# Guillaume-Helbecque/GPU-accelerated-tree-search-Chapel

Hardware: NVIDIA H100
Metric: Mnodes/s (higher is better)
Workload: dtype u8

## Files before the change

### gpu-accelerated-tree-search-chapel_b200/csrc/nq_rounds_ll.cuh

```cuda
#pragma once
#include "ll_tiers.h"
#include "nq_kernel.cuh"

namespace tsb {

constexpr int LL_T = 256;
__host__ __device__ constexpr int ll_slice(int ppt) { return LL_T * ppt; }
static_assert(ll_slice(2) == LL_SLICE2 && ll_slice(3) == LL_SLICE3, "ll_tiers.h");

enum { RND_EXIT_DONE = 0, RND_EXIT_PAUSE = 1, RND_EXIT_SPACE = 2, RND_EXIT_ABORT = 3, RND_EXIT_RELAUNCH = 4 };
struct RoundsState {
  long long size;
  unsigned epoch;
  int exit_code;
  unsigned long long rounds, parents, children, solutions;
  long long prof[12];
  long long size_hi;
  unsigned long long t_start, t_exit;
  unsigned cta_sm[LL_MAX_SMS], cta_t0[LL_MAX_SMS];
  unsigned cta_fertile[LL_MAX_SMS], cta_wide[LL_MAX_SMS];
};
__device__ __forceinline__ unsigned long long ll_globaltimer() {
  unsigned long long t;
  asm volatile("mov.u64 %0, %%globaltimer;" : "=l"(t));
  return t;
}
__device__ __forceinline__ unsigned ll_smid() {
  unsigned s;
  asm volatile("mov.u32 %0, %%smid;" : "=r"(s));
  return s;
}

__device__ __forceinline__ void st_relaxed_u64(unsigned long long* p, unsigned long long v) {
  asm volatile("st.relaxed.gpu.global.u64 [%0], %1;" ::"l"(p), "l"(v) : "memory");
}
struct SpinGuard {
  unsigned spins = 0;
  long long t0 = 0;
  __device__ __forceinline__ bool expired(unsigned* abort_flag) {
    if ((++spins & 0xFFu) != 0) return false;
    if (*reinterpret_cast<volatile unsigned*>(abort_flag)) return true;
    const long long now = clock64();
    if (t0 == 0) t0 = now;
    if (now - t0 > 4000000000LL) {
      *reinterpret_cast<volatile unsigned*>(abort_flag) = 1u;
      return true;
    }
    return false;
  }
};
constexpr int LL_CAP = 2048;
constexpr int LL_WORDS = 4;
constexpr int LL_LAYERS = 1024;
constexpr unsigned LL_TRUSTED = 0u;
__device__ __forceinline__ unsigned ll_tag(unsigned e) { return e % LL_TAG_SPAN + 1u; }

struct alignas(32) FatNode {
  unsigned long long w[LL_WORDS];
};
__device__ __forceinline__ void ll_piece(uint32_t d0, uint32_t d1, uint32_t mask, uint32_t tag, unsigned long long& a,
                                         unsigned long long& b) {
  a = static_cast<unsigned long long>(__byte_perm(mask, tag, 0x5410)) << 32 | d0;
  b = static_cast<unsigned long long>(__byte_perm(mask, tag, 0x5432)) << 32 | d1;
}
constexpr int LL_CM_SHIFT = 10;
constexpr uint32_t LL_LEAF = 1u << 30;
__host__ __device__ constexpr int ll_fw(int i) { return i / 6; }
__host__ __device__ constexpr int ll_fs(int i) { return 5 * (i % 6); }
__device__ __forceinline__ uint32_t ll_depth(uint32_t d0, uint32_t d1, uint32_t d2) {
  return d0 >> 30 | (d1 >> 30) << 2 | (d2 >> 30) << 4;
}
__device__ __forceinline__ void ll_set_depth(uint32_t (&d)[4], uint32_t depth) {
  d[0] = (d[0] & 0x3FFFFFFFu) | (depth & 3u) << 30;
  d[1] = (d[1] & 0x3FFFFFFFu) | (depth >> 2 & 3u) << 30;
  d[2] = (d[2] & 0x3FFFFFFFu) | (depth >> 4) << 30;
}
struct LlSync {
  unsigned long long slot[2][2 * LL_MAX_SMS];
  unsigned abort;
};
constexpr int LL_MAX_POOLS = 4;
struct LlParams {
  FatNode* fat;
  long long cap;
  long long size0;
  unsigned epoch0;
  unsigned epoch_last;
  int m, M;
  long long max_rounds;
  int prof;
  LlSync* sync;
  RoundsState* state;
};
struct LlMultiParams {
  LlParams pool[LL_MAX_POOLS];
};

constexpr int LL_BAR_W = 1, LL_BAR_SCAN = 2, LL_BAR_HAND = 3;
__device__ __forceinline__ void ll_bar(int threads) { asm volatile("bar.sync %0, %1;" ::"n"(LL_BAR_W), "r"(threads) : "memory"); }
__device__ __forceinline__ void ll_arrive(int id, int threads) { asm volatile("bar.arrive %0, %1;" ::"r"(id), "r"(threads) : "memory"); }
__device__ __forceinline__ void ll_wait(int id, int threads) { asm volatile("bar.sync %0, %1;" ::"r"(id), "r"(threads) : "memory"); }
__device__ __forceinline__ bool ll_bar_or(int id, int threads, bool pred) {
  uint32_t r;
  asm volatile(
      "{\n\t.reg .pred p, q;\n\t"
      "setp.ne.u32 p, %1, 0;\n\t"
      "bar.red.or.pred q, %2, %3, p;\n\t"
      "selp.u32 %0, 1, 0, q;\n\t}"
      : "=r"(r)
      : "r"(static_cast<uint32_t>(pred)), "r"(id), "r"(threads)
      : "memory");
  return r != 0;
}
__device__ __forceinline__ void ld_fat2(const unsigned long long* p, unsigned long long& a, unsigned long long& b) {
  asm volatile("ld.relaxed.gpu.global.v2.u64 {%0, %1}, [%2];" : "=l"(a), "=l"(b) : "l"(p) : "memory");
}
__device__ __forceinline__ void st_fat2(unsigned long long* p, unsigned long long a, unsigned long long b) {
  asm volatile("st.global.v2.u64 [%0], {%1, %2};" ::"l"(p), "l"(a), "l"(b));
}


__device__ __forceinline__ unsigned long long nq_aux_pack(uint32_t ld, uint32_t rd, uint32_t cm, bool leaf) {
  return static_cast<unsigned long long>(ld) | static_cast<unsigned long long>(rd) << 20 |
         static_cast<unsigned long long>(cm) << 40 | static_cast<unsigned long long>(leaf ? 1u : 0u) << 60;
}
template <int N>
__device__ __forceinline__ unsigned long long nq_aux_of_node(const uint8_t* node) {
  const int d = node[0];
  uint32_t ld = 0, rd = 0;
  for (int i = 0; i < d && i < N; i++) {
    const int b = node[1 + i], s = d - i;
    if (b + s < N) ld |= 1u << (b + s);
    if (b - s >= 0) rd |= 1u << (b - s);
  }
  const uint32_t U = ld | rd;
  uint32_t cm = 0;
  for (int k = d; k < N; k++)
    if (!((U >> (node[1 + k] & 31)) & 1u)) cm |= 1u << k;
  return nq_aux_pack(ld, rd, cm, d == N);
}
template <int N>
__global__ void nq_fat_import_kernel(const uint8_t* __restrict__ arena, FatNode* __restrict__ fat, long long size) {
  const long long p = static_cast<long long>(blockIdx.x) * blockDim.x + threadIdx.x;
  if (p >= size) return;
  const uint8_t* node = arena + p * NQ_REC;
  uint32_t d[LL_WORDS] = {0, 0, 0, 0};
  for (int i = 0; i < NQ_REC - 1; i++) d[ll_fw(i)] |= static_cast<uint32_t>(node[1 + i]) << ll_fs(i);
  ll_set_depth(d, node[0]);
  const unsigned long long aux = nq_aux_of_node<N>(node);
  d[3] |= (static_cast<uint32_t>(aux >> 40) & 0xFFFFFu) << LL_CM_SHIFT | ((aux >> 60) & 1u ? LL_LEAF : 0u);
  unsigned long long w[LL_WORDS];
  ll_piece(d[0], d[1], static_cast<uint32_t>(aux) & 0xFFFFFu, 0u, w[0], w[1]);
  ll_piece(d[2], d[3], static_cast<uint32_t>(aux >> 20) & 0xFFFFFu, 0u, w[2], w[3]);
  for (int i = 0; i < LL_WORDS; i += 2) st_fat2(&fat[p].w[i], w[i], w[i + 1]);
}
__global__ void nq_fat_clear_tags_kernel(FatNode* __restrict__ fat, long long words) {
  const long long i = static_cast<long long>(blockIdx.x) * blockDim.x + threadIdx.x;
  if (i < words) {
    unsigned long long* w = &fat[0].w[0] + i;
    *w &= 0x0000FFFFFFFFFFFFull;
  }
}
__global__ void nq_fat_export_kernel(const FatNode* __restrict__ fat, uint8_t* __restrict__ arena, long long size) {
  const long long p = static_cast<long long>(blockIdx.x) * blockDim.x + threadIdx.x;
  if (p >= size) return;
  uint8_t* node = arena + p * NQ_REC;
  uint32_t d[LL_WORDS];
  for (int i = 0; i < LL_WORDS; i++) d[i] = static_cast<uint32_t>(fat[p].w[i]);
  node[0] = static_cast<uint8_t>(ll_depth(d[0], d[1], d[2]));
  for (int i = 0; i < NQ_REC - 1; i++) node[1 + i] = static_cast<uint8_t>(d[ll_fw(i)] >> ll_fs(i) & 31u);
}

constexpr int LL_GB = 5;
__device__ __forceinline__ void ll_load_pair(const unsigned long long* p, unsigned long long& a, unsigned long long& b) {
  asm volatile("ld.relaxed.gpu.global.v2.u64 {%0, %1}, [%2];" : "=l"(a), "=l"(b) : "l"(p) : "memory");
}
static_assert(64 * LL_GB <= 2 * LL_MAX_SMS, "a lane's first LL_GB pairs lie inside LlSync::slot");
__device__ __forceinline__ bool ll_pair_carries(int n, int i, unsigned epoch, unsigned long long a, unsigned long long b) {
  return static_cast<unsigned>(a >> 32) == epoch && (i + 1 >= n || static_cast<unsigned>(b >> 32) == epoch);
}
struct LlLaneSlots {
  unsigned in, lt0, lt1;
// ... 61 lines not shown
    if (64 * u < n) {
      add(static_cast<unsigned>(v0[u]), ls.in >> (2 * u) & 1u, ls.lt0 >> (2 * u) & 1u, ls.lt1 >> (2 * u) & 1u);
      add(static_cast<unsigned>(v1[u]), ls.in >> (2 * u + 1) & 1u, ls.lt0 >> (2 * u + 1) & 1u, ls.lt1 >> (2 * u + 1) & 1u);
    }
  for (int i = c0 + 64 * LL_GB; i < n; i += 64) {
    unsigned long long a, b;
    ll_load_pair(slot + i, a, b);
    add(static_cast<unsigned>(a), true, i < k0, i < k1);
    add(static_cast<unsigned>(b), i + 1 < n, i + 1 < k0, i + 1 < k1);
  }
  all = __reduce_add_sync(0xFFFFFFFFu, all);
  before0 = __reduce_add_sync(0xFFFFFFFFu, before0);
  before1 = __reduce_add_sync(0xFFFFFFFFu, before1);
}

struct LlPlan {
  long long s0;
  int a0, len0, a1, len1;
  unsigned tag;
  int top;
  int exit;
  int off0, off1;
};
enum {
  LL_PROF_SETUP = 0, LL_PROF_POLL, LL_PROF_SCAN, LL_PROF_BUILD, LL_PROF_HAND, LL_PROF_STORE,
  LL_PROF_X_SCAN, LL_PROF_X_AHEAD, LL_PROF_X_GATHER, LL_PROF_X_TAIL, LL_PROF_X_HAND,
  LL_PROF_N
};
static_assert(LL_PROF_N <= 12, "RoundsState::prof");
template <int T, int PPT>
struct LlSmem {
  alignas(16) uint4 parent[T * PPT];
  alignas(8) uint2 diag[T * PPT];
  alignas(16) uint4 stage[LL_CAP];
  alignas(8) uint2 stage_diag[LL_CAP];
  alignas(16) uint16_t item[T * PPT * 20];
  unsigned long long warp_tot64[T / 32];
  LlPlan plan;
  int poll_abort;
  long long prof[LL_PROF_N], prof_t[2];
  unsigned prof_fertile, prof_wide;
  long long lay_start[LL_LAYERS];
  unsigned lay_tag[LL_LAYERS];
};

template <int N>
__device__ __forceinline__ uint4 ll_build_child(const uint4* parent, const uint2* diag, int item, uint2* cdiag) {
  const int r = item >> 5;
  const uint32_t k = static_cast<uint32_t>(item & 31);
  const uint4 p = parent[r];
  uint32_t P[4] = {p.x, p.y, p.z, p.w};
  const uint32_t depth = ll_depth(p.x, p.y, p.z);
  const uint32_t bd = 5u * depth + 2u * (depth * 43u >> 8), bk = 5u * k + 2u * (k * 43u >> 8);
  const auto field = [&](uint32_t b) {
    return (shr_clamp(P[0], b) | shr_clamp(P[1], b - 32u) | shr_clamp(P[2], b - 64u) | shr_clamp(P[3], b - 96u)) & 31u;
  };
  const uint32_t v = field(bk);
  const uint32_t D = field(bd) ^ v;
#pragma unroll
  for (uint32_t j = 0; j < 4; j++) P[j] ^= shl_clamp(D, bd - 32u * j) ^ shl_clamp(D, bk - 32u * j);
  const uint32_t cd = depth + 1u;
  ll_set_depth(P, cd);
  const uint2 pd = diag[r];
  const uint32_t bit = 1u << v;
  const uint32_t cld = ((pd.x | bit) << 1) & ((1u << N) - 1u), crd = (pd.y | bit) >> 1;
  *cdiag = make_uint2(cld, crd);
  const uint32_t S = ~(cld | crd);
  uint32_t cm = 0;
#pragma unroll
  for (int j = 0; j < 4; j++) {
    if (6 * j >= N) break;
    if (6 * j + 6 < N && cd >= static_cast<uint32_t>(6 * j + 6)) continue;
#pragma unroll
    for (int i = 6 * j; i < 6 * j + 6 && i < N; i++) {
      const uint32_t x = shf_r_wrap(S, 0u, P[j] >> ll_fs(i)) & 1u;
      asm("mad.lo.u32 %0, %1, %2, %0;" : "+r"(cm) : "r"(x), "r"(1u << i));
    }
  }
  cm &= shl_clamp(0xFFFFFFFFu, cd);
  P[3] = (P[3] & 0x3FFu) | cm << LL_CM_SHIFT | (cd == static_cast<uint32_t>(N) ? LL_LEAF : 0u);
  return make_uint4(P[0], P[1], P[2], P[3]);
}

template <int N, int T, int MINB, int PPT>
__global__ void __launch_bounds__(T + 32, MINB) nq_rounds_ll_kernel(const __grid_constant__ LlMultiParams mprm) {
  const LlParams& prm = mprm.pool[blockIdx.y];
  constexpr int LL_PPT = PPT;
  constexpr int TX = T + 32;
  extern __shared__ __align__(128) uint8_t smem_raw[];
  LlSmem<T, PPT>& sm = *reinterpret_cast<LlSmem<T, PPT>*>(smem_raw);
  const int t = threadIdx.x, lane = t & 31, wid = t >> 5;
  const int k = blockIdx.x, G = gridDim.x, G2 = 2 * G;
  LlSync* const sy = prm.sync;
  FatNode* const fat = prm.fat;
  const bool prof_w = prm.prof != 0 && k == 0 && t == 0;
  const bool prof_x = prm.prof != 0 && k == 0 && t == T;
#define TSB_PROF(on, who, i)          \
  if (on) {                           \
    const long long now = clock64();  \
    sm.prof[i] += now - sm.prof_t[who]; \
    sm.prof_t[who] = now;             \
  }

  long long size = prm.size0, chunk_s0 = 0, chunk_n = 0;
  long long size_hi = prm.size0;
  unsigned epoch = prm.epoch0;
  int n_lay = prm.size0 > 0 ? 1 : 0;
  long long lay_top = 0;
  unsigned long long rounds = 0, tot_parents = 0, tot_children = 0, tot_solutions = 0;
  int exit_code = RND_EXIT_PAUSE;
  long long geo_n = -1;
  int geo_a0 = 0, geo_len0 = 0, geo_a1 = 0, geo_len1 = 0;
  const auto plan = [&]() {
    int ex = -1;
    if (size < prm.m)
      ex = RND_EXIT_DONE;
    else if (static_cast<long long>(rounds) >= prm.max_rounds)
      ex = RND_EXIT_PAUSE;
    else {
      chunk_n = size < prm.M ? size : prm.M;
      chunk_s0 = size - chunk_n;
      if (chunk_s0 + chunk_n * N > prm.cap)
        ex = RND_EXIT_SPACE;
      else if (n_lay >= LL_LAYERS || epoch == prm.epoch_last)
        ex = RND_EXIT_RELAUNCH;
    }
    if (ex < 0) {
      ++epoch;
      if (chunk_n != geo_n) {
        geo_n = chunk_n;
        const unsigned n32 = static_cast<unsigned>(chunk_n), uG2 = static_cast<unsigned>(G2), uk = static_cast<unsigned>(k);
        geo_a0 = static_cast<int>(n32 * uk / uG2);
        geo_len0 = static_cast<int>(n32 * (uk + 1u) / uG2) - geo_a0;
        geo_a1 = static_cast<int>(n32 * (uG2 - 1u - uk) / uG2);
        geo_len1 = static_cast<int>(n32 * (uG2 - uk) / uG2) - geo_a1;
      }
      if (lane == 0) {
        sm.plan.s0 = chunk_s0;
        sm.plan.a0 = geo_a0;
        sm.plan.len0 = geo_len0;
        sm.plan.a1 = geo_a1;
        sm.plan.len1 = geo_len1;
        sm.plan.tag = ll_tag(epoch);
        sm.plan.top = n_lay - 1;
      }
    }
    if (lane == 0) sm.plan.exit = ex;
    return ex;
  };

  if (wid == T / 32) {
    if (lane == 0) {
      sm.lay_start[0] = 0;
      sm.lay_tag[0] = LL_TRUSTED;
      sm.poll_abort = 0;
      sm.prof_fertile = sm.prof_wide = 0;
      if (prm.prof != 0) {
        const unsigned long long now = ll_globaltimer();
        prm.state->cta_sm[k] = ll_smid();
        prm.state->cta_t0[k] = static_cast<unsigned>(now);
        if (k == 0) prm.state->t_start = now;
      }
      if (prof_x)
        for (int i = 0; i < LL_PROF_N; i++) sm.prof[i] = 0;
    }
    exit_code = plan();
  }
  __syncthreads();
  if (prm.prof != 0 && k == 0 && (t == 0 || t == T)) sm.prof_t[t == T] = clock64();

  if (wid == T / 32) {
    const LlLaneSlots lane_slots = ll_lane_slots(G2, k, G2 - 1 - k);
    while (exit_code < 0) {
      ll_wait(LL_BAR_SCAN, TX);
      TSB_PROF(prof_x, 1, LL_PROF_X_SCAN)
      if (sm.poll_abort) {
        exit_code = RND_EXIT_ABORT;
        break;
      }
      unsigned long long tot = 0;
#pragma unroll
      for (int i = 0; i < T / 32; i++) tot += sm.warp_tot64[i];
      const unsigned my_children = static_cast<unsigned>(tot & 0xFFFFF), my_leaves = static_cast<unsigned>(tot >> 20) & 0xFFFu;
      const unsigned cnt0 = static_cast<unsigned>(tot >> 32) & 0xFFFFFu;
      unsigned long long* const slots = sy->slot[epoch & 1u];
      const unsigned long long e = static_cast<unsigned long long>(epoch) << 32;
      if (lane < 2)
        st_relaxed_u64(&slots[lane == 0 ? k : G2 - 1 - k],
                       lane == 0 ? e | static_cast<unsigned long long>(my_leaves) << 20 | cnt0 : e | (my_children - cnt0));
      const long long n_prev = chunk_n;
      int nl = n_lay;
      long long below = lay_top, r_lo = 1, r_hi = 0;
      const auto plan_ahead = [&]() {
        while (nl > 0 && below >= chunk_s0) {
          --nl;
          below = nl > 0 ? sm.lay_start[nl - 1] : -1;
        }
        __syncwarp();
        if (lane == 0) {
          sm.lay_start[nl] = chunk_s0;
          sm.lay_tag[nl] = ll_tag(epoch);
          sm.plan.tag = ll_tag(epoch + 1u);
          sm.plan.top = nl;
        }
        const long long Mx = prm.M > prm.m ? prm.M : prm.m;
        r_lo = Mx - chunk_s0 > 1 ? Mx - chunk_s0 : 1;
        if (geo_n == prm.M && static_cast<long long>(rounds) + 1 < prm.max_rounds && nl + 1 < LL_LAYERS &&
            epoch != prm.epoch_last)
          r_hi = prm.cap - static_cast<long long>(prm.M) * N + prm.M - chunk_s0;
        TSB_PROF(prof_x, 1, LL_PROF_X_AHEAD)
      };
      unsigned long long v0[LL_GB], v1[LL_GB];
      const bool ok = warp_gather_slots2(slots, G2, epoch, &sy->abort, lane_slots, v0, v1, plan_ahead);
      TSB_PROF(prof_x, 1, LL_PROF_X_GATHER)
      unsigned R = 0, leaves = 0;
      if (ok) {
        unsigned before0, before1;
        warp_sum_slots2(slots, v0, v1, G2, k, G2 - 1 - k, lane_slots, R, before0, before1, leaves);
        if (lane == 0) {
          sm.plan.off0 = static_cast<int>(before0);
          sm.plan.off1 = static_cast<int>(before1);
        }
        ++rounds;
        size = chunk_s0 + R;
        n_lay = R > 0 ? nl + 1 : nl;
        lay_top = R > 0 ? chunk_s0 : below;
        if (R >= r_lo && R <= r_hi) {
          ++epoch;
          chunk_s0 = size - chunk_n;
          if (lane == 0) sm.plan.s0 = chunk_s0;
        } else {
          exit_code = plan();
        }
      }
      TSB_PROF(prof_x, 1, LL_PROF_X_TAIL)
      if (ll_bar_or(LL_BAR_HAND, TX, !ok)) {
        exit_code = RND_EXIT_ABORT;
        break;
      }
      TSB_PROF(prof_x, 1, LL_PROF_X_HAND)
      size_hi = size > size_hi ? size : size_hi;
      tot_parents += static_cast<unsigned long long>(n_prev);
      tot_children += R;
      tot_solutions += __reduce_add_sync(0xFFFFFFFFu, leaves);
    }
    if (prof_x) prm.state->t_exit = ll_globaltimer();
  } else {
    unsigned prof_fertile = 0;
    for (;;) {
      if (sm.plan.exit >= 0) break;
      const long long s0 = sm.plan.s0;
      const int a0 = sm.plan.a0, len0 = sm.plan.len0, a1 = sm.plan.a1, len1 = sm.plan.len1;
      const unsigned round_tag = sm.plan.tag;
      const int top = sm.plan.top;
      const int len = len0 + len1;
      bool ok = true;
      TSB_PROF(prof_w, 0, LL_PROF_SETUP)

      {
        SpinGuard guard;
        const unsigned long long* src0 = fat[s0 + a0].w;
        const unsigned long long* src1 = fat[s0 + a1].w - LL_WORDS * len0;
        constexpr int PCS = 2 * LL_PPT;
        unsigned long long w0[PCS], w1[PCS];
        unsigned pending = 0;
#pragma unroll
        for (int j = 0; j < PCS; j++)
          if (t + j * T < 2 * len) pending |= 1u << j;
        const long long top_start = sm.lay_start[top];
        const unsigned top_tag = sm.lay_tag[top];
        const bool in_top = s0 + min(a0, a1) >= top_start;
        const auto want_of = [&](int i) {
          if (in_top) return top_tag;
          const long long pos = s0 + (i < len0 ? a0 + i : a1 + (i - len0));
          int L = top;
          while (L > 0 && sm.lay_start[L] > pos) --L;
          return sm.lay_tag[L];
        };
        while (pending) {
#pragma unroll
          for (int j = 0; j < PCS; j++)
            if (pending & (1u << j)) {
              const int pc = t + j * T;
              ld_fat2((pc < 2 * len0 ? src0 : src1) + 2 * pc, w0[j], w1[j]);
            }
#pragma unroll
          for (int j = 0; j < PCS; j++)
            if (pending & (1u << j)) {
              const int pc = t + j * T, i = pc >> 1;
              const unsigned want = want_of(i);
              const uint32_t h0 = static_cast<uint32_t>(w0[j] >> 32), h1 = static_cast<uint32_t>(w1[j] >> 32);
              if (want == LL_TRUSTED || __byte_perm(h0, h1, 0x7632) == want * 0x10001u) {
                reinterpret_cast<uint2*>(sm.parent)[pc] = make_uint2(static_cast<uint32_t>(w0[j]), static_cast<uint32_t>(w1[j]));
                reinterpret_cast<uint32_t*>(sm.diag)[pc] = __byte_perm(h0, h1, 0x5410);
                pending &= ~(1u << j);
              }
            }
          if (pending && guard.expired(&sy->abort)) {
            ok = false;
            break;
          }
        }
      }
      if (ll_bar_or(LL_BAR_W, T, !ok)) {
        if (t == 0) sm.poll_abort = 1;
        ll_arrive(LL_BAR_SCAN, TX);
        break;
      }
      uint32_t cm[LL_PPT];
      int leaves = 0, mine = 0, mine0 = 0;
#pragma unroll
      for (int q = 0; q < LL_PPT; q++) {
        const int i = LL_PPT * t + q;
        cm[q] = 0;
        if (i < len) {
          const uint32_t w3 = sm.parent[i].w;
          cm[q] = w3 >> LL_CM_SHIFT & 0xFFFFFu;
          leaves += (w3 & LL_LEAF) ? 1 : 0;
          mine += __popc(cm[q]);
          if (i < len0) mine0 += __popc(cm[q]);
        }
      }
      TSB_PROF(prof_w, 0, LL_PROF_POLL)
      if (prm.prof != 0)
#pragma unroll
        for (int q = 0; q < LL_PPT; q++) prof_fertile += cm[q] != 0u ? 1u : 0u;
      unsigned long long incl = static_cast<unsigned long long>(mine) | static_cast<unsigned long long>(leaves) << 20 |
                                static_cast<unsigned long long>(mine0) << 32;
#pragma unroll
      for (int o = 1; o < 32; o <<= 1) {
        const unsigned long long y = __shfl_up_sync(0xFFFFFFFFu, incl, o);
        if (lane >= o) incl += y;
      }
      if (lane == 31) sm.warp_tot64[wid] = incl;
      ll_arrive(LL_BAR_SCAN, TX);
      ll_bar(T);
      unsigned long long woff = 0, tot = 0;
#pragma unroll
      for (int i = 0; i < T / 32; i++) {
        if (i < wid) woff += sm.warp_tot64[i];
        tot += sm.warp_tot64[i];
      }
      const int my_children = static_cast<int>(tot & 0xFFFFF);
      const int cnt0 = static_cast<int>(tot >> 32 & 0xFFFFF);
      if (prm.prof != 0 && t == 0 && my_children > LL_CAP) ++sm.prof_wide;
      {
        uint16_t* it = sm.item + (static_cast<int>((woff + incl) & 0xFFFFF) - mine);
#pragma unroll
        for (int q = 0; q < LL_PPT; q++) {
          uint32_t m = cm[q];
          while (m) {
            const int s = __ffs(m) - 1;
            m &= m - 1;
            *it++ = static_cast<uint16_t>(((LL_PPT * t + q) << 5) | s);
          }
        }
      }
      ll_bar(T);
      TSB_PROF(prof_w, 0, LL_PROF_SCAN)
      auto build_window = [&](int c0, int cnt) {
        for (int c = t; c < cnt; c += T)
          sm.stage[c] = ll_build_child<N>(sm.parent, sm.diag, sm.item[c0 + c], &sm.stage_diag[c]);
      };
      build_window(0, min(LL_CAP, my_children));
      TSB_PROF(prof_w, 0, LL_PROF_BUILD)
      if (ll_bar_or(LL_BAR_HAND, TX, false)) break;
      TSB_PROF(prof_w, 0, LL_PROF_HAND)
      const int off0 = sm.plan.off0, off1 = sm.plan.off1;

      for (int c0 = 0; c0 < my_children; c0 += LL_CAP) {
        const int cnt = min(LL_CAP, my_children - c0);
        if (c0 > 0) {
          ll_bar(T);
          build_window(c0, cnt);
          ll_bar(T);
        }
        unsigned long long* const dst0 = fat[s0 + off0 + c0].w;
        unsigned long long* const dst1 = fat[s0 + off1 + c0 - cnt0].w;
        const int npc = 2 * cnt;
        for (int pc = t; pc < npc; pc += 4 * T) {
          uint2 d[4];
          uint32_t dm[4];
#pragma unroll
          for (int u = 0; u < 4; u++) {
            const int x = min(pc + u * T, npc - 1);
            d[u] = reinterpret_cast<const uint2*>(sm.stage)[x];
            dm[u] = reinterpret_cast<const uint32_t*>(sm.stage_diag)[x];
          }
#pragma unroll
          for (int u = 0; u < 4; u++) {
            const int x = pc + u * T;
            unsigned long long a, b;
            ll_piece(d[u].x, d[u].y, dm[u], round_tag, a, b);
            if (x < npc) st_fat2((c0 + (x >> 1) < cnt0 ? dst0 : dst1) + 2 * x, a, b);
          }
        }
      }
      TSB_PROF(prof_w, 0, LL_PROF_STORE)
    }
    if (prm.prof != 0) atomicAdd(&sm.prof_fertile, prof_fertile);
  }
  __syncthreads();
  if (prm.prof != 0 && t == T) {
    prm.state->cta_fertile[k] = sm.prof_fertile;
    prm.state->cta_wide[k] = sm.prof_wide;
  }
  if (k == 0 && t == T) {
    RoundsState* st = prm.state;
    st->size = size;
    st->size_hi = size_hi;
    st->epoch = epoch;
    st->rounds = rounds;
    st->parents = tot_parents;
    st->children = tot_children;
    st->solutions = tot_solutions;
    st->exit_code = exit_code;
    if (prof_x)
      for (int i = 0; i < LL_PROF_N; i++) st->prof[i] = sm.prof[i];
  }
#undef TSB_PROF
}

struct RoundsSync {
  unsigned long long slot[LL_MAX_SMS];
  unsigned done[LL_MAX_SMS];
  unsigned abort;
};
__device__ __forceinline__ void st_release_u32(unsigned* p, unsigned v) {
  asm volatile("st.release.gpu.global.u32 [%0], %1;" ::"l"(p), "r"(v) : "memory");
}
template <bool CG>
__device__ __forceinline__ void bench_ld4(const unsigned* p, unsigned& v0, unsigned& v1, unsigned& v2, unsigned& v3) {
  if constexpr (CG)
    asm volatile("ld.global.cg.v4.u32 {%0, %1, %2, %3}, [%4];" : "=r"(v0), "=r"(v1), "=r"(v2), "=r"(v3) : "l"(p) : "memory");
  else
    asm volatile("ld.relaxed.gpu.global.v4.u32 {%0, %1, %2, %3}, [%4];" : "=r"(v0), "=r"(v1), "=r"(v2), "=r"(v3) : "l"(p) : "memory");
}
template <bool CG>
__device__ __forceinline__ bool bench_wait32(const unsigned* f, int G, unsigned want, unsigned* abort_flag) {
  const int lane = threadIdx.x & 31;
  SpinGuard guard;
  for (;;) {
    bool ok = true;
    for (int i = 4 * lane; i < G; i += 128) {
      unsigned v0, v1, v2, v3;
      bench_ld4<CG>(f + i, v0, v1, v2, v3);
      ok &= v0 == want && (i + 1 >= G || v1 == want) && (i + 2 >= G || v2 == want) && (i + 3 >= G || v3 == want);
    }
    if (__all_sync(0xFFFFFFFFu, ok)) return true;
    if (__any_sync(0xFFFFFFFFu, guard.expired(abort_flag))) return false;
  }
}
template <bool CG>
__device__ __forceinline__ void rounds_sync_bench_body(RoundsSync* sy, unsigned epoch0, int rounds, int variant,
                                                       uint4* scratch, long long* out_cycles) {
  const int t = threadIdx.x, wid = t >> 5, k = blockIdx.x, G = gridDim.x;
  unsigned* const slot32 = reinterpret_cast<unsigned*>(sy->slot);
  unsigned epoch = epoch0;
  const long long c0 = clock64();
  for (int r = 0; r < rounds; r++) {
    ++epoch;
    bool ok = true;
    if (!(variant & 16)) {
      if (r > 0 && wid == 0) {
        ok = bench_wait32<CG>(sy->done, G, epoch - 1u, &sy->abort);
        if (!(variant & 2)) __threadfence();
      }
      if (__syncthreads_or(!ok)) break;
    }
    if (variant & 32) {
      unsigned* const inbox = reinterpret_cast<unsigned*>(scratch) + (r & 1) * 256 * 256;
      for (int j = t; j < G; j += LL_T)
        asm volatile("st.relaxed.gpu.global.u32 [%0], %1;" ::"l"(&inbox[j * 256 + k]), "r"(epoch) : "memory");
      if (wid == 0) ok = bench_wait32<CG>(inbox + k * 256, G, epoch, &sy->abort);
      if (__syncthreads_or(!ok)) break;
      continue;
    }
    unsigned* const sl = slot32 + 256 * (r & 1);
    if (t == 0) asm volatile("st.relaxed.gpu.global.u32 [%0], %1;" ::"l"(&sl[k]), "r"(epoch) : "memory");
    if (wid == 0) ok = bench_wait32<CG>(sl, G, epoch, &sy->abort);
    if (__syncthreads_or(!ok)) break;
    if (variant & 4) __stcg(scratch + (static_cast<long long>(k) * LL_T + t), make_uint4(epoch, t, k, r));
    if (!(variant & 16)) {
      __syncthreads();
      if (t == 0) {
// ... 19 lines not shown
```

### gpu-accelerated-tree-search-chapel_b200/csrc/tsb200_api.cu

```cuda
#include <cuda_runtime.h>

#include <sched.h>

#include <algorithm>
#include <cctype>
#include <atomic>
#include <chrono>
#include <climits>
#include <cstdio>
#include <cstdlib>
#include <cstring>
#include <mutex>
#include <new>
#include <string>
#include <type_traits>
#include <vector>

#include "xfer_route.h"
#include "nq_expand.cuh"
#include "nq_rounds_ll.cuh"
#include "pfsp_expand.cuh"
#include "pfsp_rounds.cuh"
#include "nq_kernel.cuh"
#include "pfsp_kernels.cuh"
// ... 770 lines not shown
    tsb::nq_evaluate_small_kernel<N><<<grid, tsb::NQ_SMALL, 0, s>>>(in, out, static_cast<int>(count));
    TSB_CUDA(cudaGetLastError());
    h->launches++;
    return TSB_OK;
  }
  auto kernel = tsb::nq_evaluate_kernel<N>;
  const size_t smem = sizeof(tsb::NqSmem<N>) + 128;
  int grid = 1;
  int rc = h->grid_for(kernel, tsb::NQ_THREADS, smem, count, tsb::NQ_TILE, &grid);
  if (rc != TSB_OK) return rc;
  kernel<<<grid, tsb::NQ_THREADS, smem, s>>>(in, out, count);
  TSB_CUDA(cudaGetLastError());
  h->launches++;
  return TSB_OK;
}

int launch_nq(tsb_nq* h, const uint8_t* in, uint8_t* out, long long count, cudaStream_t s) {
  return with_queens(h->N, [&](auto n) { return launch_nq_n<decltype(n)::value>(h, in, out, count, s); });
}

template <int N>
int nq_expand_n(tsb_nq* h, const uint8_t* arena, const std::vector<PoolExtent>& pieces, uint8_t* children_d,
                cudaStream_t s, unsigned long long* n_children, unsigned long long* n_solutions, bool early) {
  tsb::ExpandParams prm;
  int rc = make_params(pieces, tsb::NQ_TILE, &prm);
  if (rc != TSB_OK) return rc;
  ExpandCtx& ex = h->ex;
  const bool trace = ex.epoch == 0 && std::getenv("TSB200_TRACE");
  const auto tnow = [] { return std::chrono::duration<double, std::milli>(std::chrono::steady_clock::now().time_since_epoch()).count(); };
  const double tr0 = trace ? tnow() : 0;
  rc = ex.reserve(std::max<long long>(prm.n_tiles, h->M_max / tsb::NQ_TILE + 2 * tsb::EXP_MAX_PIECES),
                  static_cast<long long>(tsb::NQ_TILE) * N * 2, s);
  if (rc != TSB_OK) return rc;
  auto k1 = tsb::nq_expand_count_kernel<N>;
  auto k3 = tsb::nq_expand_build_kernel<N>;
  const size_t smem1 = sizeof(tsb::NqCountSmem) + 128, smem3 = sizeof(tsb::NqBuildSmem) + 128;
  const long long recs = static_cast<long long>(prm.n_tiles) * tsb::NQ_TILE;
  int g1 = 1, g3 = 1;
  rc = h->grid_for(k1, tsb::NQ_THREADS, smem1, recs, tsb::NQ_TILE, &g1);
  if (rc != TSB_OK) return rc;
  rc = h->grid_for(k3, tsb::NQ_THREADS, smem3, recs, tsb::NQ_TILE, &g3);
  if (rc != TSB_OK) return rc;
  prm.epoch = ++ex.epoch;
  if ((prm.n_tiles + g3 - 1) / g3 > tsb::EXP_MAX_OWN) return TSB_EINVAL;
  uint16_t* d_items = reinterpret_cast<uint16_t*>(ex.d_cmask);
  const double tr1 = trace ? tnow() : 0;
  k1<<<g1, tsb::NQ_THREADS, smem1, s>>>(arena, prm, d_items, ex.d_tile, ex.d_st);
  k3<<<g3, tsb::NQ_THREADS, smem3, s>>>(arena, prm, d_items, ex.d_tile, children_d, ex.d_st, ex.d_res);
  TSB_CUDA(cudaGetLastError());
  h->launches += 2;
  const double tr2 = trace ? tnow() : 0;
  rc = ex.wait_result(prm.epoch, s, early);
  if (trace)
    std::fprintf(stderr, "[tsb200] first expand round: reserve+attributes %.2f ms, 2 launches %.2f ms, wait %.2f ms\n",
                 tr1 - tr0, tr2 - tr1, tnow() - tr2);
  if (rc != TSB_OK) {
    if (g_last_cuda_error.empty()) g_last_cuda_error = "expand kernels did not publish their result";
    return rc;
  }
  *n_children = ex.h_res->children;
  *n_solutions = ex.h_res->solutions;
  return TSB_OK;
}

int nq_expand(tsb_nq* h, const uint8_t* arena, const std::vector<PoolExtent>& pieces, uint8_t* children_d,
              cudaStream_t s, unsigned long long* nc, unsigned long long* ns, bool early = false) {
  return with_queens(h->N, [&](auto n) {
    return nq_expand_n<decltype(n)::value>(h, arena, pieces, children_d, s, nc, ns, early);
  });
}

bool nq_nodes_valid(int N, const tsb_nq_node* nodes, int64_t n) {
  for (int64_t i = 0; i < n; i++) {
    const tsb_nq_node& x = nodes[i];
    if (x.depth > N) return false;
    for (int j = 0; j < TSB_MAX_QUEENS; j++)
      if (x.board[j] >= (j < N ? N : 1)) return false;
  }
  return true;
}

template <int N>
int nq_ll_launch_n(tsb_nq* h, const tsb::LlMultiParams& prm, int grid, int pools, int ppt, cudaStream_t s) {
  const int var = pools == 1 ? 0 : ppt == 2 ? 1 : 2;
  auto kernel = var == 0   ? tsb::nq_rounds_ll_kernel<N, tsb::LL_T, 1, 2>
                : var == 1 ? tsb::nq_rounds_ll_kernel<N, tsb::LL_T, 2, 2>
                           : tsb::nq_rounds_ll_kernel<N, tsb::LL_T, 2, 3>;
  const size_t smem = (ppt == 2 ? sizeof(tsb::LlSmem<tsb::LL_T, 2>) : sizeof(tsb::LlSmem<tsb::LL_T, 3>)) + 128;
  int rc = h->configure(kernel, smem);
  if (rc != TSB_OK) return rc;
  void* args[] = {const_cast<tsb::LlMultiParams*>(&prm)};
  TSB_CUDA(cudaLaunchCooperativeKernel(reinterpret_cast<void*>(kernel), dim3(grid, pools), dim3(tsb::LL_T + 32), args, smem, s));
  h->launches++;
  return TSB_OK;
}
template <int N>
int nq_fat_import(tsb_nq* h) {
  const long long size = h->pool.size;
  if (size > 0) {
    tsb::nq_fat_import_kernel<N><<<static_cast<unsigned>((size + 255) / 256), 256, 0, h->stream>>>(
        h->pool.arena[h->pool.cur], h->d_fat, size);
    TSB_CUDA(cudaGetLastError());
    h->launches++;
  }
  return TSB_OK;
}
int nq_ensure_fat(tsb_nq* h, long long cap) {
  if (cap <= h->fat_cap) return TSB_OK;
  if (h->d_fat) cudaFree(h->d_fat);
  h->d_fat = nullptr;
  h->fat_cap = 0;
  TSB_CUDA(cudaMalloc(&h->d_fat, static_cast<size_t>(cap) * sizeof(tsb::FatNode)));
  h->fat_cap = cap;
  TSB_CUDA(cudaMemsetAsync(h->d_fat, 0, static_cast<size_t>(cap) * sizeof(tsb::FatNode), h->stream));
  h->tag_clear = h->rounds.epoch;
  h->tag_hi = 0;
  return TSB_OK;
}
int nq_fat_tag_window(tsb_nq* h, int64_t max_rounds, unsigned* epoch_last, bool* queued) {
  const tsb::LlTagWindow w = tsb::ll_tag_window(h->rounds.epoch, h->tag_clear, max_rounds);
  if (w.clear) {
    const long long words = h->tag_hi * tsb::LL_WORDS;
    if (words > 0) {
      tsb::nq_fat_clear_tags_kernel<<<static_cast<unsigned>((words + 255) / 256), 256, 0, h->stream>>>(h->d_fat, words);
      TSB_CUDA(cudaGetLastError());
      h->launches++;
      *queued = true;
    }
    h->tag_clear = h->rounds.epoch;
    h->tag_hi = 0;
  }
  *epoch_last = w.epoch_last;
  return TSB_OK;
}
int nq_materialize(tsb_nq* h) {
  if (!h->in_fat) return TSB_OK;
  TSB_CUDA(cudaSetDevice(h->device));
  const long long size = h->pool.size;
  if (size > 0) {
    tsb::nq_fat_export_kernel<<<static_cast<unsigned>((size + 255) / 256), 256, 0, h->stream>>>(
        h->d_fat, h->pool.arena[h->pool.cur], size);
    TSB_CUDA(cudaGetLastError());
    h->launches++;
    TSB_CUDA(cudaStreamSynchronize(h->stream));
  }
  h->in_fat = false;
  return TSB_OK;
}
int nq_ll_grid(const tsb_nq* h, int M, int pools, int* ppt = nullptr) {
  if (!h->di.coop || env_no_rounds() || pools < 1 || pools > tsb::LL_MAX_POOLS) return 0;
  const int sms = std::min(h->di.sms, tsb::LL_MAX_SMS);
  const int most = tsb::ll_ctas_per_pool(sms, pools);
  const int per = static_cast<long long>(most) * tsb::ll_slice(2) >= M ? 2 : 3;
  const int slice = tsb::ll_slice(per);
  int grid = pools == 1 ? std::max(1, (sms * 7 / 8) & ~1) : most;
  while (static_cast<long long>(grid) * slice < M && grid < most) ++grid;
  if (ppt) *ppt = per;
  return static_cast<long long>(M) <= static_cast<long long>(grid) * slice && (pools > 1 || per == 2) ? grid : 0;
}
int nq_ll_run_multi(tsb_nq* const* hs, int K, int m, int M, int64_t max_rounds, uint64_t* out) {
  int64_t left[tsb::LL_MAX_POOLS];
  bool active[tsb::LL_MAX_POOLS];
  for (int i = 0; i < K; i++) {
    left[i] = max_rounds;
    active[i] = true;
    int rc = hs[i]->rounds.ensure<tsb::LlSync>(hs[i]->stream);
    if (rc != TSB_OK) return rc;
  }
  const bool prof = std::getenv("TSB200_ROUNDS_PROF") != nullptr;
  std::vector<tsb::RoundsState> pace(prof ? tsb::LL_MAX_POOLS : 0);
  for (;;) {
    tsb::LlMultiParams mp;
    std::memset(&mp, 0, sizeof(mp));
    int map[tsb::LL_MAX_POOLS], n_act = 0;
    long long need_of[tsb::LL_MAX_POOLS];
// ... 7 lines not shown
      const long long n = std::min<long long>(p.size, M);
      const long long need = p.size - n + n * h->N;
      int rc = TSB_OK;
      if (h->in_fat && need > p.cap) rc = nq_materialize(h);
      if (rc != TSB_OK) return rc;
      bool queued = false;
      if (!h->in_fat) {
        rc = p.make_stack(h->stream, need);
        if (rc == TSB_OK) rc = nq_ensure_fat(h, p.cap);
        if (rc == TSB_OK) rc = with_queens(h->N, [h](auto q) { return nq_fat_import<decltype(q)::value>(h); });
        if (rc != TSB_OK) return rc;
        h->in_fat = true;
        queued = true;
      }
      tsb::LlParams& prm = mp.pool[n_act];
      rc = nq_fat_tag_window(h, left[i], &prm.epoch_last, &queued);
      if (rc != TSB_OK) return rc;
      if (queued && n_act > 0) TSB_CUDA(cudaStreamSynchronize(h->stream));
      prm.fat = h->d_fat;
      prm.cap = std::min(p.cap, h->fat_cap);
      prm.size0 = p.size;
      prm.epoch0 = h->rounds.epoch;
      prm.m = m;
      prm.M = M;
      prm.max_rounds = left[i];
      prm.prof = prof;
      prm.sync = h->rounds.sync<tsb::LlSync>();
      prm.state = h->rounds.d_state;
      h->rounds.h_state->exit_code = -1;
      need_of[n_act] = need;
      map[n_act++] = i;
    }
    if (n_act == 0) break;
    tsb_nq* h0 = hs[map[0]];
    int ppt = 2;
    const int grid = nq_ll_grid(h0, M, n_act, &ppt);
    if (grid == 0) return TSB_EINVAL;
    int rc = with_queens(h0->N, [&](auto q) {
      return nq_ll_launch_n<decltype(q)::value>(h0, mp, grid, n_act, ppt, h0->stream);
    });
    if (rc != TSB_OK) return rc;
    TSB_CUDA(cudaStreamSynchronize(h0->stream));
    for (int a = 0; a < n_act; a++) {
      const int i = map[a];
      tsb_nq* h = hs[i];
      tsb::RoundsState st;
      rc = h->finish_launch("nq_rounds_ll_kernel", "a flag exchange or a node poll did not complete", &st, &out[4 * i]);
      if (rc != TSB_OK) return rc;
      h->tag_hi = std::max(h->tag_hi, st.size_hi);
      if (prof) {
        const double r = static_cast<double>(std::max<unsigned long long>(1, st.rounds));
        std::fprintf(stderr, "[tsb200] LL rounds kernel (pool %d of %d): %llu rounds; CTA 0 cycles per round: workers: set-up %.0f "
                     "poll-nodes %.0f scan+items %.0f build %.0f handoff-wait %.0f store %.0f | exchange warp: "
                     "scan-wait %.0f publish+plan-ahead %.0f gather-wait %.0f sums+plan %.0f handoff-wait %.0f\n", a, n_act,
                     static_cast<unsigned long long>(st.rounds), st.prof[tsb::LL_PROF_SETUP] / r, st.prof[tsb::LL_PROF_POLL] / r,
                     st.prof[tsb::LL_PROF_SCAN] / r, st.prof[tsb::LL_PROF_BUILD] / r, st.prof[tsb::LL_PROF_HAND] / r,
                     st.prof[tsb::LL_PROF_STORE] / r, st.prof[tsb::LL_PROF_X_SCAN] / r, st.prof[tsb::LL_PROF_X_AHEAD] / r,
                     st.prof[tsb::LL_PROF_X_GATHER] / r, st.prof[tsb::LL_PROF_X_TAIL] / r, st.prof[tsb::LL_PROF_X_HAND] / r);
        pace[a] = st;
      }
      left[i] -= static_cast<int64_t>(st.rounds);
      if (st.exit_code == tsb::RND_EXIT_SPACE) {
        if (st.rounds == 0 && need_of[a] <= h->pool.cap) return TSB_ENOMEM;
        rc = nq_materialize(h);
        if (rc != TSB_OK) return rc;
      } else if (st.exit_code != tsb::RND_EXIT_RELAUNCH) {
        active[i] = false;
      }
    }
    if (prof) {
      unsigned long long t0 = ~0ull, t1 = 0;
      for (int a = 0; a < n_act; a++) {
        t0 = std::min(t0, pace[a].t_start);
        t1 = std::max(t1, pace[a].t_exit);
      }
      for (int a = 0; a < n_act; a++) {
        const tsb::RoundsState& st = pace[a];
        const double wall = 1e-3 * static_cast<double>(st.t_exit - st.t_start);
        unsigned long long fertile = 0, wide = 0;
        for (int c = 0; c < grid; c++) {
          fertile += st.cta_fertile[c];
          wide += st.cta_wide[c];
        }
        std::fprintf(stderr, "[tsb200] LL pace (pool %d of %d, handle %d): start +%.2f us, wall %.2f us, %llu rounds, "
                     "%.4f us per round, stagger %.2f us, parents %llu, children %llu, parents with children %llu, "
                     "CTA rounds over one window %llu\n", a, n_act, map[a],
                     1e-3 * static_cast<double>(st.t_start - t0), wall, static_cast<unsigned long long>(st.rounds),
                     wall / static_cast<double>(std::max<unsigned long long>(1, st.rounds)),
                     1e-3 * static_cast<double>(t1 - st.t_exit), static_cast<unsigned long long>(st.parents),
                     static_cast<unsigned long long>(st.children), fertile, wide);
      }
      int row_of[2][tsb::LL_MAX_SMS * 2], n_on[tsb::LL_MAX_SMS * 2] = {};
      unsigned t_of[2][tsb::LL_MAX_SMS * 2];
      for (int a = 0; a < n_act; a++)
        for (int c = 0; c < grid; c++) {
          const unsigned s = pace[a].cta_sm[c] % (tsb::LL_MAX_SMS * 2);
          if (n_on[s] < 2) {
            row_of[n_on[s]][s] = a;
            t_of[n_on[s]][s] = pace[a].cta_t0[c];
          }
          n_on[s]++;
        }
      int pairs[tsb::LL_MAX_POOLS][tsb::LL_MAX_POOLS] = {}, first[tsb::LL_MAX_POOLS] = {}, over = 0;
      for (int s = 0; s < tsb::LL_MAX_SMS * 2; s++) {
        if (n_on[s] > 2) over++;
        if (n_on[s] < 2) continue;
        const bool zero_first = static_cast<int>(t_of[1][s] - t_of[0][s]) >= 0;
        const int lo = std::min(row_of[0][s], row_of[1][s]), hi = std::max(row_of[0][s], row_of[1][s]);
        pairs[lo][hi]++;
        first[zero_first ? row_of[0][s] : row_of[1][s]]++;
      }
      std::string sh;
      for (int x = 0; x < n_act; x++)
        for (int y = x; y < n_act; y++)
          if (pairs[x][y]) sh += " " + std::to_string(x) + "+" + std::to_string(y) + ": " + std::to_string(pairs[x][y]);
      std::string fs;
      for (int x = 0; x < n_act; x++) fs += " " + std::to_string(x) + ": " + std::to_string(first[x]);
      std::fprintf(stderr, "[tsb200] LL residency: SMs shared by pools%s | started first on a shared SM, by pool%s | SMs "
                   "with more than two CTAs: %d\n", sh.c_str(), fs.c_str(), over);
    }
  }
  return TSB_OK;
}

template <int KIND, int M, bool SIMD>
int launch_lb1_km(tsb_pfsp* h, const uint8_t* in, uint8_t* out, long long count, cudaStream_t s) {
  auto kernel = tsb::pfsp_lb1_kernel<KIND, M, SIMD>;
  const size_t smem = sizeof(tsb::Lb1Smem) + 128;
  int grid = 1;
  int rc = h->grid_for(kernel, tsb::PF_THREADS, smem, count, tsb::PF_TILE, &grid);
  if (rc != TSB_OK) return rc;
  kernel<<<grid, tsb::PF_THREADS, smem, s>>>(in, out, count, h->d_tab1);
  TSB_CUDA(cudaGetLastError());
  h->launches++;
  return TSB_OK;
}

template <int M, typename CT>
int launch_lb2_mc(tsb_pfsp* h, const CT& C, const uint8_t* in, uint8_t* out, long long count, int best, cudaStream_t s) {
  auto kernel = tsb::pfsp_lb2_kernel<M, CT>;
  const size_t smem = sizeof(tsb::Lb2Smem<M>) + 128;
  int grid = 1;
  int rc = h->grid_for(kernel, tsb::PF_THREADS, smem, count, tsb::LB2_TILE, &grid);
  if (rc != TSB_OK) return rc;
  kernel<<<grid, tsb::PF_THREADS, smem, s>>>(in, out, count, h->d_tab1, C, best);
  TSB_CUDA(cudaGetLastError());
  h->launches++;
  return TSB_OK;
}
template <int M>
int launch_lb2_m(tsb_pfsp* h, const uint8_t* in, uint8_t* out, long long count, int best, cudaStream_t s) {
  if constexpr (M <= 10) {
    if (h->lb2u) return launch_lb2_mc<M>(h, *h->lb2u, in, out, count, best, s);
  }
  return launch_lb2_mc<M>(h, *h->lb2c, in, out, count, best, s);
}

template <int KIND, int M>
int launch_wide_km(tsb_pfsp* h, const uint8_t* in, uint8_t* out, long long count, int best, cudaStream_t s) {
  auto kernel = tsb::pfsp_wide_kernel<KIND, M>;
  const size_t smem = sizeof(tsb::PfspWideSmem) + 128;
  int grid = 1;
  int rc = h->grid_for(kernel, tsb::PW_THREADS, smem, count + tsb::PW_TILE - 1, tsb::PW_TILE, &grid);
  if (rc != TSB_OK) return rc;
  kernel<<<grid, tsb::PW_THREADS, smem, s>>>(in, reinterpret_cast<int32_t*>(out), count, h->d_wtab, best);
  TSB_CUDA(cudaGetLastError());
  h->launches++;
  return TSB_OK;
}
template <int M>
int launch_wide_m(tsb_pfsp* h, int lb_kind, const uint8_t* in, uint8_t* out, long long count, int best, cudaStream_t s) {
  if (lb_kind == TSB_LB1_D) return launch_wide_km<0, M>(h, in, out, count, best, s);
  if (lb_kind == TSB_LB1) return launch_wide_km<1, M>(h, in, out, count, best, s);
// ... 1053 lines not shown
```

Measured before the change: 34440.

## Pack two pools into one CTA using separate named barriers per half

When four pools are active, each CTA now holds two independent pool halves. Each half has its own shared-memory region and its own named-barrier IDs, so the launch uses half as many grid rows with twice the threads per block. CTA-wide __syncthreads calls become per-half named barriers so the two halves never wait on each other. The aim is to co-schedule pools on every SM deterministically instead of leaving CTA placement to the scheduler. The cost is one CTA per SM, doubled shared memory, and more pressure on named-barrier IDs.

```diff
diff --git a/gpu-accelerated-tree-search-chapel_b200/csrc/nq_rounds_ll.cuh b/gpu-accelerated-tree-search-chapel_b200/csrc/nq_rounds_ll.cuh
--- a/gpu-accelerated-tree-search-chapel_b200/csrc/nq_rounds_ll.cuh
+++ b/gpu-accelerated-tree-search-chapel_b200/csrc/nq_rounds_ll.cuh
@@ -96,8 +96,7 @@
   LlParams pool[LL_MAX_POOLS];
 };
 
-constexpr int LL_BAR_W = 1, LL_BAR_SCAN = 2, LL_BAR_HAND = 3;
-__device__ __forceinline__ void ll_bar(int threads) { asm volatile("bar.sync %0, %1;" ::"n"(LL_BAR_W), "r"(threads) : "memory"); }
+constexpr int LL_BAR_W = 1, LL_BAR_SCAN = 2, LL_BAR_HAND = 3, LL_BAR_HALF = 3;
 __device__ __forceinline__ void ll_arrive(int id, int threads) { asm volatile("bar.arrive %0, %1;" ::"r"(id), "r"(threads) : "memory"); }
 __device__ __forceinline__ void ll_wait(int id, int threads) { asm volatile("bar.sync %0, %1;" ::"r"(id), "r"(threads) : "memory"); }
 __device__ __forceinline__ bool ll_bar_or(int id, int threads, bool pred) {
@@ -325,14 +324,18 @@
   return make_uint4(P[0], P[1], P[2], P[3]);
 }
 
-template <int N, int T, int MINB, int PPT>
-__global__ void __launch_bounds__(T + 32, MINB) nq_rounds_ll_kernel(const __grid_constant__ LlMultiParams mprm) {
-  const LlParams& prm = mprm.pool[blockIdx.y];
+template <int N, int T, int MINB, int PPT, int HALVES = 1>
+__global__ void __launch_bounds__(HALVES * (T + 32), MINB) nq_rounds_ll_kernel(const __grid_constant__ LlMultiParams mprm) {
+  static_assert(HALVES == 1 || (HALVES == 2 && MINB == 1), "two pools per CTA: one CTA per SM");
   constexpr int LL_PPT = PPT;
   constexpr int TX = T + 32;
+  const int half = HALVES == 2 && threadIdx.x >= TX ? 1 : 0;
+  const LlParams& prm = mprm.pool[blockIdx.y + gridDim.y * half];
   extern __shared__ __align__(128) uint8_t smem_raw[];
-  LlSmem<T, PPT>& sm = *reinterpret_cast<LlSmem<T, PPT>*>(smem_raw);
-  const int t = threadIdx.x, lane = t & 31, wid = t >> 5;
+  LlSmem<T, PPT>& sm = reinterpret_cast<LlSmem<T, PPT>*>(smem_raw)[half];
+  const int bar_w = LL_BAR_W + LL_BAR_HALF * half, bar_scan = LL_BAR_SCAN + LL_BAR_HALF * half,
+            bar_hand = LL_BAR_HAND + LL_BAR_HALF * half;
+  const int t = threadIdx.x - TX * half, lane = t & 31, wid = t >> 5;
   const int k = blockIdx.x, G = gridDim.x, G2 = 2 * G;
   LlSync* const sy = prm.sync;
   FatNode* const fat = prm.fat;
@@ -409,13 +412,13 @@
     }
     exit_code = plan();
   }
-  __syncthreads();
+  ll_bar_or(bar_hand, TX, false);
   if (prm.prof != 0 && k == 0 && (t == 0 || t == T)) sm.prof_t[t == T] = clock64();
 
   if (wid == T / 32) {
     const LlLaneSlots lane_slots = ll_lane_slots(G2, k, G2 - 1 - k);
     while (exit_code < 0) {
-      ll_wait(LL_BAR_SCAN, TX);
+      ll_wait(bar_scan, TX);
       TSB_PROF(prof_x, 1, LL_PROF_X_SCAN)
       if (sm.poll_abort) {
         exit_code = RND_EXIT_ABORT;
@@ -477,7 +480,7 @@
         }
       }
       TSB_PROF(prof_x, 1, LL_PROF_X_TAIL)
-      if (ll_bar_or(LL_BAR_HAND, TX, !ok)) {
+      if (ll_bar_or(bar_hand, TX, !ok)) {
         exit_code = RND_EXIT_ABORT;
         break;
       }
@@ -545,9 +548,9 @@
           }
         }
       }
-      if (ll_bar_or(LL_BAR_W, T, !ok)) {
+      if (ll_bar_or(bar_w, T, !ok)) {
         if (t == 0) sm.poll_abort = 1;
-        ll_arrive(LL_BAR_SCAN, TX);
+        ll_arrive(bar_scan, TX);
         break;
       }
       uint32_t cm[LL_PPT];
@@ -576,8 +579,8 @@
         if (lane >= o) incl += y;
       }
       if (lane == 31) sm.warp_tot64[wid] = incl;
-      ll_arrive(LL_BAR_SCAN, TX);
-      ll_bar(T);
+      ll_arrive(bar_scan, TX);
+      ll_wait(bar_w, T);
       unsigned long long woff = 0, tot = 0;
 #pragma unroll
       for (int i = 0; i < T / 32; i++) {
@@ -599,7 +602,7 @@
           }
         }
       }
-      ll_bar(T);
+      ll_wait(bar_w, T);
       TSB_PROF(prof_w, 0, LL_PROF_SCAN)
       auto build_window = [&](int c0, int cnt) {
         for (int c = t; c < cnt; c += T)
@@ -607,16 +610,16 @@
       };
       build_window(0, min(LL_CAP, my_children));
       TSB_PROF(prof_w, 0, LL_PROF_BUILD)
-      if (ll_bar_or(LL_BAR_HAND, TX, false)) break;
+      if (ll_bar_or(bar_hand, TX, false)) break;
       TSB_PROF(prof_w, 0, LL_PROF_HAND)
       const int off0 = sm.plan.off0, off1 = sm.plan.off1;
 
       for (int c0 = 0; c0 < my_children; c0 += LL_CAP) {
         const int cnt = min(LL_CAP, my_children - c0);
         if (c0 > 0) {
-          ll_bar(T);
+          ll_wait(bar_w, T);
           build_window(c0, cnt);
-          ll_bar(T);
+          ll_wait(bar_w, T);
         }
         unsigned long long* const dst0 = fat[s0 + off0 + c0].w;
         unsigned long long* const dst1 = fat[s0 + off1 + c0 - cnt0].w;
@@ -643,7 +646,7 @@
     }
     if (prm.prof != 0) atomicAdd(&sm.prof_fertile, prof_fertile);
   }
-  __syncthreads();
+  ll_bar_or(bar_hand, TX, false);
   if (prm.prof != 0 && t == T) {
     prm.state->cta_fertile[k] = sm.prof_fertile;
     prm.state->cta_wide[k] = sm.prof_wide;
diff --git a/gpu-accelerated-tree-search-chapel_b200/csrc/tsb200_api.cu b/gpu-accelerated-tree-search-chapel_b200/csrc/tsb200_api.cu
--- a/gpu-accelerated-tree-search-chapel_b200/csrc/tsb200_api.cu
+++ b/gpu-accelerated-tree-search-chapel_b200/csrc/tsb200_api.cu
@@ -876,15 +876,20 @@
 
 template <int N>
 int nq_ll_launch_n(tsb_nq* h, const tsb::LlMultiParams& prm, int grid, int pools, int ppt, cudaStream_t s) {
-  const int var = pools == 1 ? 0 : ppt == 2 ? 1 : 2;
+  const int halves = pools == tsb::LL_MAX_POOLS ? 2 : 1;
+  const int var = pools == 1 ? 0 : (ppt == 2 ? 1 : 2) + (halves == 2 ? 2 : 0);
   auto kernel = var == 0   ? tsb::nq_rounds_ll_kernel<N, tsb::LL_T, 1, 2>
                 : var == 1 ? tsb::nq_rounds_ll_kernel<N, tsb::LL_T, 2, 2>
-                           : tsb::nq_rounds_ll_kernel<N, tsb::LL_T, 2, 3>;
-  const size_t smem = (ppt == 2 ? sizeof(tsb::LlSmem<tsb::LL_T, 2>) : sizeof(tsb::LlSmem<tsb::LL_T, 3>)) + 128;
+                : var == 2 ? tsb::nq_rounds_ll_kernel<N, tsb::LL_T, 2, 3>
+                : var == 3 ? tsb::nq_rounds_ll_kernel<N, tsb::LL_T, 1, 2, 2>
+                           : tsb::nq_rounds_ll_kernel<N, tsb::LL_T, 1, 3, 2>;
+  static_assert(2 * sizeof(tsb::LlSmem<tsb::LL_T, 3>) + 128 <= 227 * 1024, "two halves' shared memory in one CTA");
+  const size_t smem = halves * (ppt == 2 ? sizeof(tsb::LlSmem<tsb::LL_T, 2>) : sizeof(tsb::LlSmem<tsb::LL_T, 3>)) + 128;
   int rc = h->configure(kernel, smem);
   if (rc != TSB_OK) return rc;
   void* args[] = {const_cast<tsb::LlMultiParams*>(&prm)};
-  TSB_CUDA(cudaLaunchCooperativeKernel(reinterpret_cast<void*>(kernel), dim3(grid, pools), dim3(tsb::LL_T + 32), args, smem, s));
+  TSB_CUDA(cudaLaunchCooperativeKernel(reinterpret_cast<void*>(kernel), dim3(grid, pools / halves),
+                                       dim3(halves * (tsb::LL_T + 32)), args, smem, s));
   h->launches++;
   return TSB_OK;
 }
@@ -1058,13 +1063,16 @@
           fertile += st.cta_fertile[c];
           wide += st.cta_wide[c];
         }
+        static const char* const why[] = {"dry", "budget", "space", "abort", "relaunch"};
         std::fprintf(stderr, "[tsb200] LL pace (pool %d of %d, handle %d): start +%.2f us, wall %.2f us, %llu rounds, "
                      "%.4f us per round, stagger %.2f us, parents %llu, children %llu, parents with children %llu, "
-                     "CTA rounds over one window %llu\n", a, n_act, map[a],
+                     "CTA rounds over one window %llu, exit %s, globaltimer %llu..%llu ns\n", a, n_act, map[a],
                      1e-3 * static_cast<double>(st.t_start - t0), wall, static_cast<unsigned long long>(st.rounds),
                      wall / static_cast<double>(std::max<unsigned long long>(1, st.rounds)),
                      1e-3 * static_cast<double>(t1 - st.t_exit), static_cast<unsigned long long>(st.parents),
-                     static_cast<unsigned long long>(st.children), fertile, wide);
+                     static_cast<unsigned long long>(st.children), fertile, wide,
+                     st.exit_code >= 0 && st.exit_code <= tsb::RND_EXIT_RELAUNCH ? why[st.exit_code] : "?", st.t_start,
+                     st.t_exit);
       }
       int row_of[2][tsb::LL_MAX_SMS * 2], n_on[tsb::LL_MAX_SMS * 2] = {};
       unsigned t_of[2][tsb::LL_MAX_SMS * 2];
```

New measurement: 35470 (median of 6 runs). 1.03x the previous value.
